# PantoMatrix/PantoMatrix

Hardware: NVIDIA H100
Metric: motion_frames_per_sec (higher is better)
Workload: dtype fp16x3 (two fp16 operand planes, 3 products, f32 accumulate)

## Files before the change

### pantomatrix_b200/csrc/pm_attention_tc.cu

```cuda
#include "pm_common.cuh"
#include "pm_tc_ptx.cuh"
#include "../../include/pm_emage.h"

namespace {

constexpr int T = 64;
constexpr int HD = 192;
constexpr int KB = HD / 64;
constexpr int BLK = T * 128;
constexpr int NTHREADS = 128;
constexpr float P_SCALE = 1024.f;

struct Smem {
  static constexpr int Q = 0;
  static constexpr int K = Q + 2 * KB * BLK;
  static constexpr int V = K + 2 * KB * BLK;
  static constexpr int P = V + 2 * KB * BLK;
  static constexpr int BARS = P + 2 * BLK;
  static constexpr int TOTAL = BARS + (KB + 1) * 8;
};

#ifdef PM_ATTN_TIMING
__device__ unsigned long long pm_attn_stamps[16];
#define AT_STAMP(i) do { if (blockIdx.x == 0 && (threadIdx.x & 31) == 0) pm_attn_stamps[i] = (unsigned long long)clock64(); } while (0)
#else
#define AT_STAMP(i) do {} while (0)
#endif

struct AttnParams {
  int heads, tq, tk;
  int qc0, kc0, vc0;
  float scale;
  float* out; int ldo;
  PmPlanes planes;
};

__global__ void __launch_bounds__(NTHREADS, 1) attention_tc_kernel(const __grid_constant__ CUtensorMap map_q,
                                                                   const __grid_constant__ CUtensorMap map_k,
                                                                   const __grid_constant__ CUtensorMap map_v,
                                                                   const AttnParams p) {
  extern __shared__ __align__(1024) uint8_t smem_raw[];
  uint8_t* sm = reinterpret_cast<uint8_t*>((reinterpret_cast<uintptr_t>(smem_raw) + 1023) & ~uintptr_t(1023));
  const uint32_t sm_u = smem_u32(sm);
  const uint32_t bars = sm_u + Smem::BARS;
  const uint32_t qk_full = bars, v_full = bars + 8 * KB;
  const int warp = threadIdx.x >> 5, lane = threadIdx.x & 31;
  const int b = blockIdx.x / p.heads, h = blockIdx.x % p.heads;
  if (warp == 0) AT_STAMP(0);

  if (threadIdx.x == 0) {
    for (int kb = 0; kb < KB; ++kb) mbar_init(qk_full + 8 * kb, 1);
    mbar_init(v_full, 1);
    asm volatile("fence.mbarrier_init.release.cluster;" ::: "memory");
  }
  __syncthreads();
  if (warp == 0) AT_STAMP(1);
  if (warp == 0) {
    if (elect_one()) {
      asm volatile("prefetch.tensormap [%0];" ::"l"(&map_q) : "memory");
      asm volatile("prefetch.tensormap [%0];" ::"l"(&map_k) : "memory");
      asm volatile("prefetch.tensormap [%0];" ::"l"(&map_v) : "memory");
      for (int kb = 0; kb < KB; ++kb) {
        mbar_expect_tx(qk_full + 8 * kb, 4 * BLK);
        for (int pl = 0; pl < 2; ++pl) {
          tma_load_4d(sm_u + Smem::Q + (pl * KB + kb) * BLK, &map_q, qk_full + 8 * kb, p.qc0 + h * HD + kb * 64, 0, b, pl);
          tma_load_4d(sm_u + Smem::K + (pl * KB + kb) * BLK, &map_k, qk_full + 8 * kb, p.kc0 + h * HD + kb * 64, 0, b, pl);
        }
      }
      mbar_expect_tx(v_full, 2 * KB * BLK);
      for (int pl = 0; pl < 2; ++pl)
        for (int nb = 0; nb < KB; ++nb)
          tma_load_4d(sm_u + Smem::V + (pl * KB + nb) * BLK, &map_v, v_full, p.vc0 + h * HD + nb * 64, 0, b, pl);
    }
    __syncwarp();
  }

  const int r0 = warp * 16 + (lane >> 2), t2 = 2 * (lane & 3);
  const int pa[3] = {0, 1, 0}, pb[3] = {1, 0, 0};

  float sr[32];
#pragma unroll
  for (int i = 0; i < 32; ++i) sr[i] = 0.f;
#pragma unroll
  for (int kb = 0; kb < KB; ++kb) {
    mbar_wait(qk_full + 8 * kb, 0);
    if (warp == 0) AT_STAMP(8 + kb);
    wgmma_fence();
#pragma unroll
// ... 126 lines not shown
}

extern "C" int pm_attention_tc(const uint16_t* Q, long long q_ps, long long q_bs, int ldq, int q_cols, int q_col0,
                               const uint16_t* K, long long k_ps, long long k_bs, int ldk, int k_cols, int k_col0,
                               const uint16_t* V, long long v_ps, long long v_bs, int ldv, int v_cols, int v_col0,
                               float* O, int ldo, int batch, int heads, int tq, int tk, int head_dim,
                               uint16_t* planes, long long p_ps, int p_ld, int p_nsplit, void* stream) {
  PM_REQUIRE(Q && K && V && (O || planes) && batch >= 0 && heads > 0);
  PM_TAKE_FMT(p_nsplit, f16);
  PM_REQUIRE(!planes || (f16 && p_nsplit <= 2));
  PM_REQUIRE(pm_planes_ok(planes, p_ps, p_ld, p_nsplit, heads * head_dim, false));
  if (head_dim != HD || tq > T || tk > T || tq <= 0 || tk <= 0) return PM_EUNSUPPORTED;
  PM_REQUIRE(!O || (ldo & 3) == 0);
  for (const void* ptr : {(const void*)Q, (const void*)K, (const void*)V}) PM_REQUIRE((reinterpret_cast<uintptr_t>(ptr) & 15) == 0);
  PM_REQUIRE((ldq & 7) == 0 && (ldk & 7) == 0 && (ldv & 7) == 0 && (q_ps & 7) == 0 && (k_ps & 7) == 0 && (v_ps & 7) == 0);
  PM_REQUIRE(batch <= 1 || ((q_bs & 7) == 0 && (k_bs & 7) == 0 && (v_bs & 7) == 0));
  PM_REQUIRE(q_col0 >= 0 && k_col0 >= 0 && v_col0 >= 0 && q_col0 + heads * HD <= q_cols && k_col0 + heads * HD <= k_cols &&
             v_col0 + heads * HD <= v_cols && q_cols <= ldq && k_cols <= ldk && v_cols <= ldv);
  if (batch == 0) return PM_OK;
  CUtensorMap mq, mk, mv;
  if (!plane_map(&mq, Q, q_ps, q_bs, ldq, q_cols, tq, batch) || !plane_map(&mk, K, k_ps, k_bs, ldk, k_cols, tk, batch) ||
      !plane_map(&mv, V, v_ps, v_bs, ldv, v_cols, tk, batch))
    return PM_EBADARG;
  AttnParams p;
  p.heads = heads; p.tq = tq; p.tk = tk; p.qc0 = q_col0; p.kc0 = k_col0; p.vc0 = v_col0;
  p.scale = 1.0f / (sqrtf((float)head_dim) * PM_F16_ACT_SCALE * PM_F16_ACT_SCALE);
  p.out = O; p.ldo = ldo;
  p.planes = PmPlanes{reinterpret_cast<__nv_bfloat16*>(planes), p_ps, p_ld, p_nsplit};
  static unsigned long long configured = 0;
  if (pm_first_use_on_device(configured)) {
    cudaError_t e = cudaFuncSetAttribute(attention_tc_kernel, cudaFuncAttributeMaxDynamicSharedMemorySize, (int)kSmem);
    if (e != cudaSuccess) { configured = 0; return (int)e; }
  }
  attention_tc_kernel<<<batch * heads, NTHREADS, kSmem, (cudaStream_t)stream>>>(mq, mk, mv, p);
  PM_LAUNCH_CHECK();
}

#ifdef PM_ATTN_TIMING
extern "C" int pm_attn_timing_read(unsigned long long* host) {
  cudaError_t e = cudaDeviceSynchronize();
  if (e != cudaSuccess) return (int)e;
  return (int)cudaMemcpyFromSymbol(host, pm_attn_stamps, sizeof(unsigned long long) * 16);
}
#endif
```

### pantomatrix_b200/csrc/pm_common.cuh

```cuda
#pragma once
#include <cuda_bf16.h>
#include <cuda_fp16.h>
#include <cuda_runtime.h>
#include <stdint.h>

#define PM_OK 0
#define PM_EBADARG (-1)
#define PM_EUNSUPPORTED (-2)

#define PM_LAUNCH_CHECK()                                  \
  do {                                                     \
    cudaError_t _e = cudaGetLastError();                   \
    return _e == cudaSuccess ? PM_OK : (int)_e;            \
  } while (0)

#define PM_REQUIRE(cond) \
  do {                   \
    if (!(cond)) return PM_EBADARG; \
  } while (0)

static inline int pm_cdiv(long long a, long long b) { return (int)((a + b - 1) / b); }

static inline bool pm_first_use_on_device(unsigned long long& mask) {
  int d = 0;
  if (cudaGetDevice(&d) != cudaSuccess || d < 0 || d >= 64) return true;
  if ((mask >> d) & 1ull) return false;
  mask |= 1ull << d;
  return true;
}

enum PmAct { PM_ACT_NONE = 0, PM_ACT_RELU = 1, PM_ACT_LEAKY = 2 };

__device__ __forceinline__ float pm_act(float v, int act, float slope) {
  if (act == PM_ACT_RELU) return v > 0.f ? v : 0.f;
  if (act == PM_ACT_LEAKY) return v > 0.f ? v : v * slope;
  return v;
}

__device__ __forceinline__ float pm_warp_sum(float v) {
#pragma unroll
  for (int o = 16; o > 0; o >>= 1) v += __shfl_xor_sync(0xffffffffu, v, o);
  return v;
}

__device__ __forceinline__ float pm_warp_max(float v) {
#pragma unroll
  for (int o = 16; o > 0; o >>= 1) v = fmaxf(v, __shfl_xor_sync(0xffffffffu, v, o));
  return v;
}

struct PmPlanes {
  __nv_bfloat16* ptr;
  long long ps;
  int ld;
// ... 99 lines not shown
```

### pantomatrix_b200/csrc/pm_elementwise.cu

```cuda
#include "pm_common.cuh"
#include "../../include/pm_emage.h"

namespace {

constexpr int STEM_ROWS = 192;
constexpr int STEM_THREADS = 256;

template <bool F16>
__device__ __forceinline__ void stem_store_planes2(const PmPlanes& P, long long row, int c, float a, float b) {
  if constexpr (F16) {
    if (P.nsplit == 2) {
      __half* o = reinterpret_cast<__half*>(P.ptr) + row * P.ld + c;
      a *= PM_F16_ACT_SCALE; b *= PM_F16_ACT_SCALE;
      const float a0 = pm_f16_head(a), b0 = pm_f16_head(b);
      *reinterpret_cast<__half2*>(o) = __floats2half2_rn(a0, b0);
      *reinterpret_cast<__half2*>(o + P.ps) = __floats2half2_rn(a - a0, b - b0);
      return;
    }
  }
  pm_store_planes_t<F16>(P, row, c, a);
  pm_store_planes_t<F16>(P, row, c + 1, b);
}

template <int KS, int COUT, bool F16>
// ... 54 lines not shown
      }
    } else {
#pragma unroll
      for (int j = 0; j < 3; ++j) {
#pragma unroll
        for (int k = 0; k < KS; ++k) {
          const float v = xr[j * stride + k];
          acc[j][0] = fmaf(v, wa0[k], acc[j][0]);
          acc[j][1] = fmaf(v, wa1[k], acc[j][1]);
          acc[j][2] = fmaf(v, wb0[k], acc[j][2]);
          acc[j][3] = fmaf(v, wb1[k], acc[j][3]);
        }
      }
    }
#pragma unroll
    for (int j = 0; j < 3; ++j) {
      const int l = l0 + r0 + j;
      if (l >= rows_out) break;
      float a0 = acc[j][0] + ba0, a1 = acc[j][1] + ba1;
      a0 = a0 > 0.f ? a0 : a0 * slope;
      a1 = a1 > 0.f ? a1 : a1 * slope;
      const long long row = (long long)seq * rows_out + l;
      *reinterpret_cast<float2*>(sc + row * COUT + c0) = make_float2(acc[j][2] + bb0, acc[j][3] + bb1);
      if (y1) *reinterpret_cast<float2*>(y1 + row * COUT + c0) = make_float2(a0, a1);
      if (P.ptr) stem_store_planes2<F16>(P, row, c0, a0, a1);
    }
  }
}

template <int VEC, bool F16>
__global__ void __launch_bounds__(256) add_layernorm_kernel(
    const float* __restrict__ x, const float* __restrict__ r, const float* __restrict__ gamma,
    const float* __restrict__ beta, float* __restrict__ out, long long rows, float eps, PmPlanes P) {
  const int lane = threadIdx.x & 31;
  const long long row = (long long)blockIdx.x * (blockDim.x >> 5) + (threadIdx.x >> 5);
  if (row >= rows) return;
  constexpr int CH = VEC * 128;
  const float4* __restrict__ xr = reinterpret_cast<const float4*>(x + row * CH);
  const float4* __restrict__ rr = r ? reinterpret_cast<const float4*>(r + row * CH) : nullptr;
  float4 v[VEC];
  float s = 0.f;
#pragma unroll
  for (int i = 0; i < VEC; ++i) {
    v[i] = xr[lane + 32 * i];
    if (rr) {
      const float4 t = rr[lane + 32 * i];
      v[i].x += t.x; v[i].y += t.y; v[i].z += t.z; v[i].w += t.w;
    }
    s += (v[i].x + v[i].y) + (v[i].z + v[i].w);
  }
  const float mean = pm_warp_sum(s) * (1.f / CH);
  float q = 0.f;
#pragma unroll
  for (int i = 0; i < VEC; ++i) {
    const float a = v[i].x - mean, b = v[i].y - mean, c = v[i].z - mean, d = v[i].w - mean;
    q += (a * a + b * b) + (c * c + d * d);
  }
  const float rstd = rsqrtf(pm_warp_sum(q) * (1.f / CH) + eps);
  const float4* __restrict__ g4 = reinterpret_cast<const float4*>(gamma);
  const float4* __restrict__ b4 = reinterpret_cast<const float4*>(beta);
  float4* __restrict__ o4 = out ? reinterpret_cast<float4*>(out + row * CH) : nullptr;
#pragma unroll
  for (int i = 0; i < VEC; ++i) {
    const float4 g = g4[lane + 32 * i], bb = b4[lane + 32 * i];
    float4 o;
    o.x = (v[i].x - mean) * rstd * g.x + bb.x;
    o.y = (v[i].y - mean) * rstd * g.y + bb.y;
    o.z = (v[i].z - mean) * rstd * g.z + bb.z;
    o.w = (v[i].w - mean) * rstd * g.w + bb.w;
    if (o4) o4[lane + 32 * i] = o;
    if (P.ptr) pm_store_planes4_t<F16>(P, row, (lane + 32 * i) * 4, o);
  }
}

__device__ __forceinline__ float4 pick_row(int code, const float* pe, const float* spk, int b, int t, int ch, int c4) {
  if (code == 1) return reinterpret_cast<const float4*>(pe + (long long)t * ch)[c4];
  if (code == 2) return reinterpret_cast<const float4*>(spk + (long long)b * ch)[c4];
  return make_float4(0.f, 0.f, 0.f, 0.f);
}

template <bool F16>
__global__ void __launch_bounds__(256) add_rows_kernel(
    const float* __restrict__ x, const float* __restrict__ pe, const float* __restrict__ spk,
    int first, int second, float* __restrict__ out, int batch, int rows, int ch, PmPlanes P) {
  const int ch4 = ch >> 2;
  const long long total = (long long)batch * rows * ch4;
  for (long long i = (long long)blockIdx.x * blockDim.x + threadIdx.x; i < total;
       i += (long long)gridDim.x * blockDim.x) {
    const int c4 = (int)(i % ch4);
    const long long bt = i / ch4;
    const int t = (int)(bt % rows), b = (int)(bt / rows);
    float4 v = x ? reinterpret_cast<const float4*>(x)[i] : make_float4(0.f, 0.f, 0.f, 0.f);
    if (first) {
      const float4 a = pick_row(first, pe, spk, b, t, ch, c4);
      v.x += a.x; v.y += a.y; v.z += a.z; v.w += a.w;
    }
    if (second) {
      const float4 a = pick_row(second, pe, spk, b, t, ch, c4);
      v.x += a.x; v.y += a.y; v.z += a.z; v.w += a.w;
    }
    if (out) reinterpret_cast<float4*>(out)[i] = v;
    if (P.ptr) pm_store_planes4_t<F16>(P, bt, c4 * 4, v);
  }
}

template <bool F16>
__global__ void __launch_bounds__(256) add2_kernel(const float* __restrict__ a, long long lda,
                                                   const float* __restrict__ b, long long ldb,
                                                   float* __restrict__ out, long long ldo, long long rows,
                                                   long long ch, long long nv, PmPlanes P) {
  const long long i0 = (long long)blockIdx.x * blockDim.x + threadIdx.x, step = (long long)gridDim.x * blockDim.x;
  for (long long i = i0; i < rows * nv; i += step) {
    const long long r = rows == 1 ? 0 : i / nv, c = (i - r * nv) * 4;
    const float4 u = *reinterpret_cast<const float4*>(a + r * lda + c);
    const float4 v = *reinterpret_cast<const float4*>(b + r * ldb + c);
    const float4 o = make_float4(u.x + v.x, u.y + v.y, u.z + v.z, u.w + v.w);
    if (out) *reinterpret_cast<float4*>(out + r * ldo + c) = o;
    if (P.ptr) pm_store_planes4_t<F16>(P, r, (int)c, o);
  }
  const long long nt = ch - 4 * nv;
  for (long long i = i0; i < rows * nt; i += step) {
    const long long r = i / nt, c = 4 * nv + (i - r * nt);
    const float o = a[r * lda + c] + b[r * ldb + c];
    if (out) out[r * ldo + c] = o;
    if (P.ptr) pm_store_planes_t<F16>(P, r, (int)c, o);
  }
}

template <bool F16>
__global__ void __launch_bounds__(256) window_input_kernel(
    const float* __restrict__ motion, const float* __restrict__ mask, const float* __restrict__ seed,
    const float* __restrict__ mask_embedding, float* __restrict__ out,
    int batch, int total_len, int start, int win_len, int pre, int ch, long long seed_bs, PmPlanes P) {
  const long long total = (long long)batch * win_len * ch;
  for (long long i = (long long)blockIdx.x * blockDim.x + threadIdx.x; i < total;
       i += (long long)gridDim.x * blockDim.x) {
    const int c = (int)(i % ch);
    const long long bf = i / ch;
    const int f = (int)(bf % win_len), b = (int)(bf / win_len);
    const long long src = ((long long)b * total_len + start + f) * ch + c;
    float m = mask ? mask[src] : 1.f;
    float v = motion ? motion[src] : ((c < ch - 7 && (c % 6 == 0 || c % 6 == 4)) ? 1.f : 0.f);
    if (f < pre) {
      if (m != 0.f && seed) v = seed[(long long)b * seed_bs + (long long)f * ch + c];
      m = 0.f;
    }
    const float o = (m == 1.f) ? mask_embedding[c] : v;
    if (out) out[i] = o;
    if (P.ptr) pm_store_planes_t<F16>(P, bf, c, o);
  }
}

inline int grid_for(long long work, int threads) {
  long long g = (work + threads - 1) / threads;
  const long long cap = 148LL * 16;
  return (int)(g < 1 ? 1 : (g > cap ? cap : g));
}

}

extern "C" int pm_wav_stem_f32(const float* audio, long long a_bs, long long a_ws, int batch, int windows,
                               int n_samples, const float* w1, const float* b1, const float* wd,
                               const float* bd, int cout, int ksize, int stride, int pad, int rows_out,
                               float slope, float* y1, float* sc,
                               uint16_t* planes, long long p_ps, int p_ld, int p_nsplit, void* stream) {
  PM_REQUIRE(audio && w1 && b1 && wd && bd && sc && (y1 || planes));
  PM_REQUIRE(batch > 0 && windows > 0 && n_samples > 0 && cout > 0 && stride > 0 && rows_out > 0);
  PM_TAKE_FMT(p_nsplit, f16);
  PM_REQUIRE(pm_planes_ok(planes, p_ps, p_ld, p_nsplit, cout, false));
  PM_REQUIRE(!planes || ((p_ld & 1) == 0 && (p_ps & 1) == 0 && (reinterpret_cast<uintptr_t>(planes) & 3) == 0));
  PM_REQUIRE((reinterpret_cast<uintptr_t>(sc) & 7) == 0 && (!y1 || (reinterpret_cast<uintptr_t>(y1) & 7) == 0));
  if (ksize != 15 || (cout != 32 && cout != 64)) return PM_EUNSUPPORTED;
  PM_REQUIRE((long long)batch * windows <= 65535);
  const size_t smem = (size_t)((STEM_ROWS - 1) * stride + ksize) * sizeof(float);
  PM_REQUIRE(smem <= 48 * 1024);
  const PmPlanes P{reinterpret_cast<__nv_bfloat16*>(planes), p_ps, p_ld, planes ? p_nsplit : 0};
  dim3 grid(pm_cdiv(rows_out, STEM_ROWS), batch * windows);
  cudaStream_t st = (cudaStream_t)stream;
#define PM_STEM(CO, F)                                                                                          \
  wav_stem_kernel<15, CO, F><<<grid, STEM_THREADS, smem, st>>>(audio, a_bs, a_ws, batch, n_samples, w1, b1, wd, bd, \
                                                               stride, pad, rows_out, slope, y1, sc, P)
  if (cout == 64) { if (f16) PM_STEM(64, true); else PM_STEM(64, false); }
  else { if (f16) PM_STEM(32, true); else PM_STEM(32, false); }
#undef PM_STEM
  PM_LAUNCH_CHECK();
}

extern "C" int pm_add_layernorm_f32(const float* x, const float* r, const float* gamma, const float* beta,
                                    float* out, long long rows, int ch, float eps,
                                    uint16_t* planes, long long p_ps, int p_ld, int p_nsplit, void* stream) {
  PM_REQUIRE(x && gamma && beta && (out || planes) && rows >= 0);
  PM_TAKE_FMT(p_nsplit, f16);
  PM_REQUIRE(pm_planes_ok(planes, p_ps, p_ld, p_nsplit, ch, true));
  const PmPlanes P{reinterpret_cast<__nv_bfloat16*>(planes), p_ps, p_ld, p_nsplit};
  if (rows == 0) return PM_OK;
  const int warps = 8;
  const unsigned grid = (unsigned)((rows + warps - 1) / warps);
  cudaStream_t st = (cudaStream_t)stream;
  switch (ch) {
    case 256:
      if (f16) add_layernorm_kernel<2, true><<<grid, warps * 32, 0, st>>>(x, r, gamma, beta, out, rows, eps, P);
      else add_layernorm_kernel<2, false><<<grid, warps * 32, 0, st>>>(x, r, gamma, beta, out, rows, eps, P);
      break;
    case 512:
      if (f16) add_layernorm_kernel<4, true><<<grid, warps * 32, 0, st>>>(x, r, gamma, beta, out, rows, eps, P);
      else add_layernorm_kernel<4, false><<<grid, warps * 32, 0, st>>>(x, r, gamma, beta, out, rows, eps, P);
      break;
    case 768:
      if (f16) add_layernorm_kernel<6, true><<<grid, warps * 32, 0, st>>>(x, r, gamma, beta, out, rows, eps, P);
      else add_layernorm_kernel<6, false><<<grid, warps * 32, 0, st>>>(x, r, gamma, beta, out, rows, eps, P);
      break;
    case 1024:
      if (f16) add_layernorm_kernel<8, true><<<grid, warps * 32, 0, st>>>(x, r, gamma, beta, out, rows, eps, P);
      else add_layernorm_kernel<8, false><<<grid, warps * 32, 0, st>>>(x, r, gamma, beta, out, rows, eps, P);
      break;
    default: return PM_EUNSUPPORTED;
  }
  PM_LAUNCH_CHECK();
}

extern "C" int pm_add_rows_f32(const float* x, const float* pe, const float* spk, int first, int second,
                               float* out, int batch, int rows, int ch,
                               uint16_t* planes, long long p_ps, int p_ld, int p_nsplit, void* stream) {
  PM_REQUIRE((out || planes) && batch >= 0 && rows >= 0 && ch > 0 && (ch & 3) == 0);
  PM_TAKE_FMT(p_nsplit, f16);
  PM_REQUIRE(pm_planes_ok(planes, p_ps, p_ld, p_nsplit, ch, true));
  const PmPlanes P{reinterpret_cast<__nv_bfloat16*>(planes), p_ps, p_ld, p_nsplit};
  PM_REQUIRE(first >= 0 && first <= 2 && second >= 0 && second <= 2);
  PM_REQUIRE((first != 1 && second != 1) || pe);
  PM_REQUIRE((first != 2 && second != 2) || spk);
  const long long total = (long long)batch * rows * (ch >> 2);
  if (total == 0) return PM_OK;
  if (f16) add_rows_kernel<true><<<grid_for(total, 256), 256, 0, (cudaStream_t)stream>>>(x, pe, spk, first, second, out,
                                                                                  batch, rows, ch, P);
  else add_rows_kernel<false><<<grid_for(total, 256), 256, 0, (cudaStream_t)stream>>>(x, pe, spk, first, second, out,
                                                                               batch, rows, ch, P);
  PM_LAUNCH_CHECK();
}

extern "C" int pm_add2_strided_f32(const float* a, long long lda, const float* b, long long ldb, float* out,
                                   long long ldo, long long rows, long long ch,
                                   uint16_t* planes, long long p_ps, int p_ld, int p_nsplit, void* stream) {
  PM_REQUIRE(a && b && (out || planes) && rows >= 0 && ch > 0);
  PM_REQUIRE(rows <= 1 || (lda >= ch && ldb >= ch && (!out || ldo >= ch)));
  PM_REQUIRE(!planes || ((ch & 3) == 0 && ch <= 0x7fffffffLL));
  PM_TAKE_FMT(p_nsplit, f16);
  PM_REQUIRE(pm_planes_ok(planes, p_ps, p_ld, p_nsplit, (int)(planes ? ch : 1), true));
  const PmPlanes P{reinterpret_cast<__nv_bfloat16*>(planes), p_ps, p_ld, p_nsplit};
  if (rows == 0) return PM_OK;
  const auto a16 = [](const void* p) { return (reinterpret_cast<uintptr_t>(p) & 15) == 0; };
  const bool vec = a16(a) && a16(b) && (!out || a16(out)) &&
                   (rows == 1 || ((lda & 3) == 0 && (ldb & 3) == 0 && (!out || (ldo & 3) == 0)));
  const long long nv = vec ? ch / 4 : 0;
  const int grid = grid_for(rows * (nv + (ch - 4 * nv)), 256);
  cudaStream_t st = (cudaStream_t)stream;
  if (f16) add2_kernel<true><<<grid, 256, 0, st>>>(a, lda, b, ldb, out, ldo, rows, ch, nv, P);
  else add2_kernel<false><<<grid, 256, 0, st>>>(a, lda, b, ldb, out, ldo, rows, ch, nv, P);
  PM_LAUNCH_CHECK();
}

extern "C" int pm_add2_f32(const float* a, const float* b, float* out, long long n, int ch,
                           uint16_t* planes, long long p_ps, int p_ld, int p_nsplit, void* stream) {
  PM_REQUIRE(a && b && (out || planes) && n >= 0);
  PM_REQUIRE(!planes || (ch > 0 && (ch & 3) == 0 && n % ch == 0));
  if (n == 0) return PM_OK;
  const long long rows = planes ? n / ch : 1, cols = planes ? ch : n;
  return pm_add2_strided_f32(a, cols, b, cols, out, cols, rows, cols, planes, p_ps, p_ld, p_nsplit, stream);
}

extern "C" int pm_window_input_f32(const float* motion, const float* mask, const float* seed,
                                   const float* mask_embedding, float* out, int batch, int total_len,
                                   int start, int win_len, int pre, int ch, long long seed_bs,
                                   uint16_t* planes, long long p_ps, int p_ld, int p_nsplit, void* stream) {
  PM_REQUIRE(mask_embedding && (out || planes));
  PM_TAKE_FMT(p_nsplit, f16);
  PM_REQUIRE(pm_planes_ok(planes, p_ps, p_ld, p_nsplit, ch, false));
  const PmPlanes P{reinterpret_cast<__nv_bfloat16*>(planes), p_ps, p_ld, p_nsplit};
  PM_REQUIRE(batch >= 0 && win_len >= 0 && start >= 0 && start + win_len <= total_len && pre >= 0 && ch > 0);
  const long long total = (long long)batch * win_len * ch;
  if (total == 0) return PM_OK;
  if (f16) window_input_kernel<true><<<grid_for(total, 256), 256, 0, (cudaStream_t)stream>>>(
      motion, mask, seed, mask_embedding, out, batch, total_len, start, win_len, pre, ch, seed_bs, P);
  else window_input_kernel<false><<<grid_for(total, 256), 256, 0, (cudaStream_t)stream>>>(
      motion, mask, seed, mask_embedding, out, batch, total_len, start, win_len, pre, ch, seed_bs, P);
  PM_LAUNCH_CHECK();
}
```

### pantomatrix_b200/csrc/pm_tapgemm_tc.cu

```cuda
#include <cuda.h>
#include <stdio.h>
#include <stdlib.h>

#include <cstring>
#include "pm_common.cuh"
#include "../../include/pm_emage.h"


namespace {

constexpr int BM = 128;
constexpr int BK = 64;
constexpr int MMA_K = 16;
constexpr int A_TILE_BYTES = BM * BK * 2;
constexpr int PRODUCER_THREADS = 128;
constexpr int CONSUMER_THREADS = 256;
constexpr int NUM_THREADS = PRODUCER_THREADS + CONSUMER_THREADS;
constexpr int PRODUCER_REGS = 40, CONSUMER_REGS = 232;
static_assert(PRODUCER_THREADS * PRODUCER_REGS + CONSUMER_THREADS * CONSUMER_REGS == (65536 / NUM_THREADS & ~7) * NUM_THREADS,
              "the setmaxnreg split must use exactly the launch's register pool");
constexpr int STAMP_WARP = PRODUCER_THREADS / 32;
constexpr int MAX_STAGES = 8;
constexpr int RING_KB = 200;

// ... 74 lines not shown
  const int warp = threadIdx.x >> 5, lane = threadIdx.x & 31;
  if (warp == STAMP_WARP) PM_STAMP(0);
  const int l0 = blockIdx.x * p.R;
  const int n0 = blockIdx.y * BN;
  const int b0 = blockIdx.z * p.NB;
  const int n_iter = p.taps * p.kblocks;

  if (threadIdx.x == 0) {
    asm volatile("prefetch.tensormap [%0];" ::"l"(&map_a) : "memory");
    asm volatile("prefetch.tensormap [%0];" ::"l"(&map_w) : "memory");
    for (int s = 0; s < p.stages; ++s) {
      mbar_init(smem_u32(&full_bar[s]), 1);
      mbar_init(smem_u32(&empty_bar[s]), 2);
    }
    asm volatile("fence.mbarrier_init.release.cluster;" ::: "memory");
  }
  __syncthreads();
  if (warp == STAMP_WARP) PM_STAMP(1);

  if (warp < PRODUCER_THREADS / 32) {
    setmaxnreg_dec<PRODUCER_REGS>();
    if (warp == 1 && lane == 0 && p.prefetch) {
      const long long ncta = (long long)gridDim.x * gridDim.y * gridDim.z;
      const long long cta = ((long long)blockIdx.z * gridDim.y + blockIdx.y) * gridDim.x + blockIdx.x;
      long long share = ((p.prefetch_bytes + ncta - 1) / ncta + 127) & ~127LL;
      long long off = cta * share;
      long long end = off + share < p.prefetch_bytes ? off + share : p.prefetch_bytes;
      end &= ~15LL;
      for (; off < end; off += 16384) {
        const uint32_t n = (uint32_t)(end - off < 16384 ? end - off : 16384);
        asm volatile("cp.async.bulk.prefetch.L2.global [%0], %1;" ::"l"(p.prefetch + off), "r"(n) : "memory");
      }
    }
    if (warp != 0) return;
    const uint32_t tx = (uint32_t)stage_bytes;
    int s = 0, tap = 0, kb = 0;
    uint32_t ph = 0;
    for (int it = 0; it < n_iter; ++it) {
      mbar_wait_fast(smem_u32(&empty_bar[s]), ph ^ 1u);
      if (elect_one()) {
        const uint32_t bar = smem_u32(&full_bar[s]);
        uint8_t* st = tiles + (size_t)s * stage_bytes;
        mbar_expect_tx(bar, tx);
        for (int pl = 0; pl < p.nsplit; ++pl) {
          tma_load_4d(smem_u32(st + pl * A_TILE_BYTES), &map_a, bar, kb * BK, l0 + tap - p.pad, b0, pl);
          tma_load_3d(smem_u32(st + p.nsplit * A_TILE_BYTES + pl * W_TILE_BYTES), &map_w, bar, kb * BK, tap * p.w_rows + n0, pl);
        }
      }
      __syncwarp();
      if (++s == p.stages) { s = 0; ph ^= 1u; }
      if (++kb == p.kblocks) { kb = 0; ++tap; }
    }
    return;
  }

  setmaxnreg_inc<CONSUMER_REGS>();
  const int ct = threadIdx.x - PRODUCER_THREADS;
  const int wg = ct >> 7;
  float acc0[NACC], acc1[NACC], accc[NACC];
#pragma unroll
  for (int i = 0; i < NACC; ++i) { acc0[i] = 0.f; acc1[i] = 0.f; accc[i] = 0.f; }
  {
    const uint32_t tiles_u32 = smem_u32(tiles);
    int s = 0;
    uint32_t ph = 0;
    int prev = -1;
    auto kblock = [&](float (&main)[NACC]) {
      mbar_wait_fast(smem_u32(&full_bar[s]), ph);
      if (prev < 0 && warp == STAMP_WARP) PM_STAMP(2);
      const uint32_t a_base = tiles_u32 + (uint32_t)s * (uint32_t)stage_bytes + (uint32_t)wg * (64 * 128);
      const uint32_t w_base = tiles_u32 + (uint32_t)s * (uint32_t)stage_bytes + (uint32_t)(NSPLIT * A_TILE_BYTES);
      wgmma_fence();
      mma_kblock<BN, F16, NSPLIT>(main, accc, gmma_desc(GMMA_DESC_K_SW128, a_base), gmma_desc(GMMA_DESC_K_SW128, w_base));
      wgmma_commit();
      wgmma_wait<1>();
      if (prev >= 0 && ct % 128 == 0) mbar_arrive(smem_u32(&empty_bar[prev]));
      prev = s;
      if (++s == p.stages) { s = 0; ph ^= 1u; }
    };
    int it = 0;
    for (; it + 1 < n_iter; it += 2) {
      kblock(acc0);
      kblock(acc1);
    }
    if (it < n_iter) kblock(acc0);
    if (warp == STAMP_WARP) PM_STAMP(3);
    wgmma_wait<0>();
    if (warp == STAMP_WARP) PM_STAMP(4);
    wgmma_fence_regs(acc0);
    wgmma_fence_regs(acc1);
    wgmma_fence_regs(accc);
  }
  named_bar_sync(1, CONSUMER_THREADS);
  {
    const int wq = warp & 3, t4 = lane & 3;
    const int r0 = wg * 64 + wq * 16 + (lane >> 2);
    float* stg = reinterpret_cast<float*>(tiles);
#pragma unroll
    for (int i = 0; i < NACC / 4; ++i) {
      const int c = 8 * i + 2 * t4;
#pragma unroll
      for (int h = 0; h < 2; ++h) {
        float v0 = acc0[4 * i + 2 * h] + acc1[4 * i + 2 * h];
        float v1 = acc0[4 * i + 2 * h + 1] + acc1[4 * i + 2 * h + 1];
        v0 += accc[4 * i + 2 * h];
        v1 += accc[4 * i + 2 * h + 1];
        if constexpr (F16) { v0 *= p.acc_scale; v1 *= p.acc_scale; }
        *reinterpret_cast<float2*>(stg + (r0 + 8 * h) * ST + c) = make_float2(v0, v1);
      }
    }
  }
  named_bar_sync(1, CONSUMER_THREADS);

  const bool vec_f = p.out_f32 && ((p.ldo & 3) == 0) && ((reinterpret_cast<uintptr_t>(p.out_f32) & 15) == 0) && ((p.o_bs & 3) == 0);
  const bool vec_r = p.residual && ((p.ldr & 3) == 0) && ((reinterpret_cast<uintptr_t>(p.residual) & 15) == 0) && ((p.r_bs & 3) == 0);
  const bool vec_b = p.out_bf16 && ((p.ldob & 3) == 0) && ((reinterpret_cast<uintptr_t>(p.out_bf16) & 7) == 0) &&
                     ((p.ob_bs & 3) == 0) && ((p.ob_ps & 3) == 0);
  const bool all_vec = (!p.out_f32 || vec_f) && (!p.residual || vec_r) && (!p.out_bf16 || vec_b);
  const float act_slope = p.act == PM_ACT_NONE ? 1.f : (p.act == PM_ACT_RELU ? 0.f : p.slope);
  const int r_shift = 31 - __clz(p.R);
  constexpr int C4 = BN / 4;
  const float* stg = reinterpret_cast<const float*>(tiles);
#pragma unroll 1
  for (int item = ct; item < BM * C4; item += CONSUMER_THREADS) {
    const int rt = item / C4, c = (item % C4) * 4;
    const int b = b0 + (rt >> r_shift), l = l0 + (rt & (p.R - 1));
    const int n = n0 + c;
    if (b >= p.batch || l >= p.rows_out || n >= p.cout) continue;
    const float4 x4 = *reinterpret_cast<const float4*>(stg + rt * ST + c);
    const long long of = (long long)b * p.o_bs + (long long)l * p.ldo;
    const long long orr = (long long)b * p.r_bs + (long long)l * p.ldr;
    const PmPlanes P{p.out_bf16 ? p.out_bf16 + (long long)b * p.ob_bs + (long long)l * p.ldob : nullptr,
                     p.ob_ps, p.ldob, p.out_nsplit};
    if (all_vec && n + 4 <= p.cout) {
      float4 x = x4;
      if (p.bias) { x.x += __ldg(p.bias + n); x.y += __ldg(p.bias + n + 1); x.z += __ldg(p.bias + n + 2); x.w += __ldg(p.bias + n + 3); }
      if (p.residual) {
        const float4 t = *reinterpret_cast<const float4*>(p.residual + orr + n);
        x.x += t.x; x.y += t.y; x.z += t.z; x.w += t.w;
      }
      x.x = x.x < 0.f ? (n < p.act_cols ? act_slope : 1.f) * x.x : x.x;
      x.y = x.y < 0.f ? (n + 1 < p.act_cols ? act_slope : 1.f) * x.y : x.y;
      x.z = x.z < 0.f ? (n + 2 < p.act_cols ? act_slope : 1.f) * x.z : x.z;
      x.w = x.w < 0.f ? (n + 3 < p.act_cols ? act_slope : 1.f) * x.w : x.w;
      if (p.out_f32) *reinterpret_cast<float4*>(p.out_f32 + of + n) = x;
      if (P.ptr) pm_store_planes4_t<F16>(P, 0, n, x);
    } else {
      const float xs[4] = {x4.x, x4.y, x4.z, x4.w};
#pragma unroll
      for (int k = 0; k < 4; ++k) {
        if (n + k >= p.cout) break;
        float y = xs[k];
        if (p.bias) y += __ldg(p.bias + n + k);
        if (p.residual) y += p.residual[orr + n + k];
        y = y < 0.f ? (n + k < p.act_cols ? act_slope : 1.f) * y : y;
        if (p.out_f32) p.out_f32[of + n + k] = y;
        if (P.ptr) pm_store_planes_t<F16>(P, 0, n + k, y);
      }
    }
  }
  if (warp == STAMP_WARP) PM_STAMP(5);
#ifdef PM_TC_TIMING
  named_bar_sync(1, CONSUMER_THREADS);
#endif
  if (warp == STAMP_WARP) PM_STAMP(6);
}

template <bool VEC, bool F16>
__global__ void __launch_bounds__(256) split_bf16_kernel(const float* __restrict__ x, long long x_bs, int ldx, int rows,
                                                         int ch, __nv_bfloat16* __restrict__ out, long long o_ps,
                                                         long long o_bs, int ldo, int nsplit) {
  const int b = blockIdx.y;
  const float* __restrict__ xb = x + (long long)b * x_bs;
  __nv_bfloat16* __restrict__ ob = out + (long long)b * o_bs;
  if (VEC) {
    const int ch4 = ch >> 2;
    const long long total = (long long)rows * ch4;
    for (long long i = (long long)blockIdx.x * blockDim.x + threadIdx.x; i < total; i += (long long)gridDim.x * blockDim.x) {
      const int r = (int)(i / ch4), c4 = (int)(i - (long long)r * ch4);
      const float4 v = *reinterpret_cast<const float4*>(xb + (long long)r * ldx + 4 * c4);
      const PmPlanes P{ob, o_ps, ldo, nsplit};
      pm_store_planes4_t<F16>(P, r, 4 * c4, v);
    }
  } else {
    const long long total = (long long)rows * ch;
    for (long long i = (long long)blockIdx.x * blockDim.x + threadIdx.x; i < total; i += (long long)gridDim.x * blockDim.x) {
      const int r = (int)(i / ch), c = (int)(i - (long long)r * ch);
      const PmPlanes P{ob, o_ps, ldo, nsplit};
      pm_store_planes_t<F16>(P, r, c, xb[(long long)r * ldx + c]);
    }
  }
}

template <int BN, bool F16, int NSPLIT>
int launch(const CUtensorMap& ma, const CUtensorMap& mw, TcParams& p, dim3 grid, cudaStream_t st) {
  const int stage_bytes = p.nsplit * (A_TILE_BYTES + BN * BK * 2);
  int stages = RING_KB * 1024 / stage_bytes;
  if (stages > MAX_STAGES) stages = MAX_STAGES;
  if (stages < 2) return PM_EUNSUPPORTED;
  p.stages = stages;
  const int staging = BM * (BN + 8) * 4;
  const size_t ring = (size_t)stages * stage_bytes > (size_t)staging ? (size_t)stages * stage_bytes : (size_t)staging;
  const size_t smem = ring + 1024  + 2 * MAX_STAGES * sizeof(uint64_t);
  static unsigned long long configured = 0;
  if (pm_first_use_on_device(configured)) {
    cudaError_t e = cudaFuncSetAttribute(tapgemm_tc_kernel<BN, F16, NSPLIT>, cudaFuncAttributeMaxDynamicSharedMemorySize, 227 * 1024);
    if (e != cudaSuccess) { configured = 0; return (int)e; }
  }
  tapgemm_tc_kernel<BN, F16, NSPLIT><<<grid, NUM_THREADS, smem, st>>>(ma, mw, p);
  PM_LAUNCH_CHECK();
}

template <int BN>
int launch_fmt(const CUtensorMap& ma, const CUtensorMap& mw, TcParams& p, dim3 grid, cudaStream_t st, bool f16) {
  if (f16) {
    if (p.nsplit == 1) return launch<BN, true, 1>(ma, mw, p, grid, st);
    if (p.nsplit == 2) return launch<BN, true, 2>(ma, mw, p, grid, st);
    return launch<BN, true, 3>(ma, mw, p, grid, st);
  }
  if (p.nsplit == 1) return launch<BN, false, 1>(ma, mw, p, grid, st);
  if (p.nsplit == 2) return launch<BN, false, 2>(ma, mw, p, grid, st);
  return launch<BN, false, 3>(ma, mw, p, grid, st);
}

int pick_bn(long long row_tiles, int cout, int w_rows, int sms) {
  if (cout <= 64 || w_rows % 128) return 64;
  const long long waves64 = (row_tiles * pm_cdiv(cout, 64) + sms - 1) / sms;
  const long long waves128 = (row_tiles * pm_cdiv(cout, 128) + sms - 1) / sms;
  return waves128 * 14 <= waves64 * 10 ? 128 : 64;
}

}

extern "C" int pm_tapgemm_tc(const uint16_t* A, long long a_ps, long long a_bs, int lda, int batch, int rows_in, int cin,
                             const uint16_t* W, long long w_ps, int w_rows, int ldw, int taps, int pad, int nsplit,
                             const float* bias, int rows_out, int cout,
                             const float* residual, long long r_bs, int ldr,
                             int act, int act_cols, float slope, float acc_scale,
                             float* out_f32, long long o_bs, int ldo,
                             uint16_t* out_bf16, long long ob_ps, long long ob_bs, int ldob, int out_nsplit,
                             const void* prefetch, long long prefetch_bytes, void* stream) {
  PM_REQUIRE(A && W && (out_f32 || out_bf16));
// ... 63 lines not shown
}

#ifdef PM_TC_TIMING
extern "C" int pm_tc_timing_reset() {
  cudaError_t e = cudaDeviceSynchronize();
  if (e != cudaSuccess) return (int)e;
  void* d = nullptr;
  e = cudaGetSymbolAddress(&d, pm_tc_stamps);
  if (e != cudaSuccess) return (int)e;
  return (int)cudaMemset(d, 0, sizeof(unsigned long long) * 4096 * 8);
}
extern "C" int pm_tc_timing_read(unsigned long long* host) {
  cudaError_t e = cudaDeviceSynchronize();
  if (e != cudaSuccess) return (int)e;
  return (int)cudaMemcpyFromSymbol(host, pm_tc_stamps, sizeof(unsigned long long) * 4096 * 8);
}
#endif

extern "C" int pm_split_bf16(const float* x, long long x_bs, int ldx, int batch, int rows, int ch,
                             uint16_t* out, long long o_ps, long long o_bs, int ldo, int nsplit, void* stream) {
  PM_TAKE_FMT(nsplit, f16);
  PM_REQUIRE(x && out && batch >= 0 && rows >= 0 && ch > 0 && ldx >= ch && ldo >= ch && nsplit >= 1 && nsplit <= 3);
  if ((long long)batch * rows == 0) return PM_OK;
  PM_REQUIRE(batch <= 65535);
  const bool vec = (ch & 3) == 0 && (ldx & 3) == 0 && (x_bs & 3) == 0 && (ldo & 3) == 0 && (o_bs & 3) == 0 &&
                   (o_ps & 3) == 0 && (reinterpret_cast<uintptr_t>(x) & 15) == 0 && (reinterpret_cast<uintptr_t>(out) & 7) == 0;
  const long long work = (long long)rows * (vec ? ch / 4 : ch);
  long long gx = (work + 255) / 256;
  const long long cap = batch >= 132 * 4 ? 1 : (132 * 8 + batch - 1) / batch;
  if (gx > cap) gx = cap;
  dim3 grid((unsigned)gx, batch);
  __nv_bfloat16* o = reinterpret_cast<__nv_bfloat16*>(out);
  cudaStream_t st = (cudaStream_t)stream;
  if (f16) {
    if (vec) split_bf16_kernel<true, true><<<grid, 256, 0, st>>>(x, x_bs, ldx, rows, ch, o, o_ps, o_bs, ldo, nsplit);
    else split_bf16_kernel<false, true><<<grid, 256, 0, st>>>(x, x_bs, ldx, rows, ch, o, o_ps, o_bs, ldo, nsplit);
  } else {
    if (vec) split_bf16_kernel<true, false><<<grid, 256, 0, st>>>(x, x_bs, ldx, rows, ch, o, o_ps, o_bs, ldo, nsplit);
    else split_bf16_kernel<false, false><<<grid, 256, 0, st>>>(x, x_bs, ldx, rows, ch, o, o_ps, o_bs, ldo, nsplit);
  }
  PM_LAUNCH_CHECK();
}
```

Measured before the change: 304,700.

## Enable programmatic dependent launch across kernels and prefetch GEMM weights before wait

Launches the attention, elementwise, split and tap-GEMM kernels with programmatic stream serialization and adds griddepcontrol wait/trigger calls. Each kernel's prologue (barrier init, tensormap prefetch, weight TMA loads for the first stages) can then overlap the tail of the previous kernel. The GEMM producer issues weight tile loads before waiting on the upstream kernel, because weights do not depend on prior outputs. The epilogue is also restructured so each thread keeps one column, hoisting the bias load and batching the residual loads. The risk is a correctness hazard if any prologue touches data written by the predecessor, and the extra launch-attribute overhead.

```diff
diff --git a/pantomatrix_b200/csrc/pm_attention_tc.cu b/pantomatrix_b200/csrc/pm_attention_tc.cu
--- a/pantomatrix_b200/csrc/pm_attention_tc.cu
+++ b/pantomatrix_b200/csrc/pm_attention_tc.cu
@@ -54,6 +54,8 @@
     asm volatile("fence.mbarrier_init.release.cluster;" ::: "memory");
   }
   __syncthreads();
+  pm_pdl_wait();
+  pm_pdl_trigger();
   if (warp == 0) AT_STAMP(1);
   if (warp == 0) {
     if (elect_one()) {
@@ -246,7 +248,7 @@
     cudaError_t e = cudaFuncSetAttribute(attention_tc_kernel, cudaFuncAttributeMaxDynamicSharedMemorySize, (int)kSmem);
     if (e != cudaSuccess) { configured = 0; return (int)e; }
   }
-  attention_tc_kernel<<<batch * heads, NTHREADS, kSmem, (cudaStream_t)stream>>>(mq, mk, mv, p);
+  pm_launch_pdl(attention_tc_kernel, dim3(batch * heads), dim3(NTHREADS), kSmem, (cudaStream_t)stream, mq, mk, mv, p);
   PM_LAUNCH_CHECK();
 }
 
diff --git a/pantomatrix_b200/csrc/pm_common.cuh b/pantomatrix_b200/csrc/pm_common.cuh
--- a/pantomatrix_b200/csrc/pm_common.cuh
+++ b/pantomatrix_b200/csrc/pm_common.cuh
@@ -20,6 +20,25 @@
   } while (0)
 
 static inline int pm_cdiv(long long a, long long b) { return (int)((a + b - 1) / b); }
+
+__device__ __forceinline__ void pm_pdl_wait() { asm volatile("griddepcontrol.wait;" ::: "memory"); }
+__device__ __forceinline__ void pm_pdl_trigger() { asm volatile("griddepcontrol.launch_dependents;" ::: "memory"); }
+
+template <typename... KArgs, typename... Args>
+static inline cudaError_t pm_launch_pdl(void (*kernel)(KArgs...), dim3 grid, dim3 block, size_t smem, cudaStream_t st,
+                                        Args&&... args) {
+  cudaLaunchAttribute attr[1];
+  attr[0].id = cudaLaunchAttributeProgrammaticStreamSerialization;
+  attr[0].val.programmaticStreamSerializationAllowed = 1;
+  cudaLaunchConfig_t cfg = {};
+  cfg.gridDim = grid;
+  cfg.blockDim = block;
+  cfg.dynamicSmemBytes = smem;
+  cfg.stream = st;
+  cfg.attrs = attr;
+  cfg.numAttrs = 1;
+  return cudaLaunchKernelEx(&cfg, kernel, static_cast<Args&&>(args)...);
+}
 
 static inline bool pm_first_use_on_device(unsigned long long& mask) {
   int d = 0;
diff --git a/pantomatrix_b200/csrc/pm_elementwise.cu b/pantomatrix_b200/csrc/pm_elementwise.cu
--- a/pantomatrix_b200/csrc/pm_elementwise.cu
+++ b/pantomatrix_b200/csrc/pm_elementwise.cu
@@ -110,6 +110,8 @@
 __global__ void __launch_bounds__(256) add_layernorm_kernel(
     const float* __restrict__ x, const float* __restrict__ r, const float* __restrict__ gamma,
     const float* __restrict__ beta, float* __restrict__ out, long long rows, float eps, PmPlanes P) {
+  pm_pdl_wait();
+  pm_pdl_trigger();
   const int lane = threadIdx.x & 31;
   const long long row = (long long)blockIdx.x * (blockDim.x >> 5) + (threadIdx.x >> 5);
   if (row >= rows) return;
@@ -161,6 +163,8 @@
 __global__ void __launch_bounds__(256) add_rows_kernel(
     const float* __restrict__ x, const float* __restrict__ pe, const float* __restrict__ spk,
     int first, int second, float* __restrict__ out, int batch, int rows, int ch, PmPlanes P) {
+  pm_pdl_wait();
+  pm_pdl_trigger();
   const int ch4 = ch >> 2;
   const long long total = (long long)batch * rows * ch4;
   for (long long i = (long long)blockIdx.x * blockDim.x + threadIdx.x; i < total;
@@ -187,6 +191,8 @@
                                                    const float* __restrict__ b, long long ldb,
                                                    float* __restrict__ out, long long ldo, long long rows,
                                                    long long ch, long long nv, PmPlanes P) {
+  pm_pdl_wait();
+  pm_pdl_trigger();
   const long long i0 = (long long)blockIdx.x * blockDim.x + threadIdx.x, step = (long long)gridDim.x * blockDim.x;
   for (long long i = i0; i < rows * nv; i += step) {
     const long long r = rows == 1 ? 0 : i / nv, c = (i - r * nv) * 4;
@@ -210,6 +216,8 @@
     const float* __restrict__ motion, const float* __restrict__ mask, const float* __restrict__ seed,
     const float* __restrict__ mask_embedding, float* __restrict__ out,
     int batch, int total_len, int start, int win_len, int pre, int ch, long long seed_bs, PmPlanes P) {
+  pm_pdl_wait();
+  pm_pdl_trigger();
   const long long total = (long long)batch * win_len * ch;
   for (long long i = (long long)blockIdx.x * blockDim.x + threadIdx.x; i < total;
        i += (long long)gridDim.x * blockDim.x) {
@@ -275,25 +283,23 @@
   const int warps = 8;
   const unsigned grid = (unsigned)((rows + warps - 1) / warps);
   cudaStream_t st = (cudaStream_t)stream;
+  void (*kern)(const float*, const float*, const float*, const float*, float*, long long, float, PmPlanes);
   switch (ch) {
     case 256:
-      if (f16) add_layernorm_kernel<2, true><<<grid, warps * 32, 0, st>>>(x, r, gamma, beta, out, rows, eps, P);
-      else add_layernorm_kernel<2, false><<<grid, warps * 32, 0, st>>>(x, r, gamma, beta, out, rows, eps, P);
+      kern = f16 ? add_layernorm_kernel<2, true> : add_layernorm_kernel<2, false>;
       break;
     case 512:
-      if (f16) add_layernorm_kernel<4, true><<<grid, warps * 32, 0, st>>>(x, r, gamma, beta, out, rows, eps, P);
-      else add_layernorm_kernel<4, false><<<grid, warps * 32, 0, st>>>(x, r, gamma, beta, out, rows, eps, P);
+      kern = f16 ? add_layernorm_kernel<4, true> : add_layernorm_kernel<4, false>;
       break;
     case 768:
-      if (f16) add_layernorm_kernel<6, true><<<grid, warps * 32, 0, st>>>(x, r, gamma, beta, out, rows, eps, P);
-      else add_layernorm_kernel<6, false><<<grid, warps * 32, 0, st>>>(x, r, gamma, beta, out, rows, eps, P);
+      kern = f16 ? add_layernorm_kernel<6, true> : add_layernorm_kernel<6, false>;
       break;
     case 1024:
-      if (f16) add_layernorm_kernel<8, true><<<grid, warps * 32, 0, st>>>(x, r, gamma, beta, out, rows, eps, P);
-      else add_layernorm_kernel<8, false><<<grid, warps * 32, 0, st>>>(x, r, gamma, beta, out, rows, eps, P);
+      kern = f16 ? add_layernorm_kernel<8, true> : add_layernorm_kernel<8, false>;
       break;
     default: return PM_EUNSUPPORTED;
   }
+  pm_launch_pdl(kern, dim3(grid), dim3(warps * 32), 0, st, x, r, gamma, beta, out, rows, eps, P);
   PM_LAUNCH_CHECK();
 }
 
@@ -309,10 +315,8 @@
   PM_REQUIRE((first != 2 && second != 2) || spk);
   const long long total = (long long)batch * rows * (ch >> 2);
   if (total == 0) return PM_OK;
-  if (f16) add_rows_kernel<true><<<grid_for(total, 256), 256, 0, (cudaStream_t)stream>>>(x, pe, spk, first, second, out,
-                                                                                  batch, rows, ch, P);
-  else add_rows_kernel<false><<<grid_for(total, 256), 256, 0, (cudaStream_t)stream>>>(x, pe, spk, first, second, out,
-                                                                               batch, rows, ch, P);
+  pm_launch_pdl(f16 ? add_rows_kernel<true> : add_rows_kernel<false>, dim3(grid_for(total, 256)), dim3(256), 0,
+                (cudaStream_t)stream, x, pe, spk, first, second, out, batch, rows, ch, P);
   PM_LAUNCH_CHECK();
 }
 
@@ -332,8 +336,8 @@
   const long long nv = vec ? ch / 4 : 0;
   const int grid = grid_for(rows * (nv + (ch - 4 * nv)), 256);
   cudaStream_t st = (cudaStream_t)stream;
-  if (f16) add2_kernel<true><<<grid, 256, 0, st>>>(a, lda, b, ldb, out, ldo, rows, ch, nv, P);
-  else add2_kernel<false><<<grid, 256, 0, st>>>(a, lda, b, ldb, out, ldo, rows, ch, nv, P);
+  pm_launch_pdl(f16 ? add2_kernel<true> : add2_kernel<false>, dim3(grid), dim3(256), 0, st, a, lda, b, ldb, out, ldo, rows,
+                ch, nv, P);
   PM_LAUNCH_CHECK();
 }
 
@@ -357,9 +361,8 @@
   PM_REQUIRE(batch >= 0 && win_len >= 0 && start >= 0 && start + win_len <= total_len && pre >= 0 && ch > 0);
   const long long total = (long long)batch * win_len * ch;
   if (total == 0) return PM_OK;
-  if (f16) window_input_kernel<true><<<grid_for(total, 256), 256, 0, (cudaStream_t)stream>>>(
-      motion, mask, seed, mask_embedding, out, batch, total_len, start, win_len, pre, ch, seed_bs, P);
-  else window_input_kernel<false><<<grid_for(total, 256), 256, 0, (cudaStream_t)stream>>>(
-      motion, mask, seed, mask_embedding, out, batch, total_len, start, win_len, pre, ch, seed_bs, P);
-  PM_LAUNCH_CHECK();
-}
+  pm_launch_pdl(f16 ? window_input_kernel<true> : window_input_kernel<false>, dim3(grid_for(total, 256)), dim3(256), 0,
+                (cudaStream_t)stream, motion, mask, seed, mask_embedding, out, batch, total_len, start, win_len, pre, ch,
+                seed_bs, P);
+  PM_LAUNCH_CHECK();
+}
diff --git a/pantomatrix_b200/csrc/pm_tapgemm_tc.cu b/pantomatrix_b200/csrc/pm_tapgemm_tc.cu
--- a/pantomatrix_b200/csrc/pm_tapgemm_tc.cu
+++ b/pantomatrix_b200/csrc/pm_tapgemm_tc.cu
@@ -130,8 +130,25 @@
         asm volatile("cp.async.bulk.prefetch.L2.global [%0], %1;" ::"l"(p.prefetch + off), "r"(n) : "memory");
       }
     }
-    if (warp != 0) return;
+    if (warp != 0) {
+      pm_pdl_wait();
+      return;
+    }
     const uint32_t tx = (uint32_t)stage_bytes;
+    const int pre = n_iter < p.stages ? n_iter : p.stages;
+    if (elect_one()) {
+      int tap = 0, kb = 0;
+      for (int it = 0; it < pre; ++it) {
+        const uint32_t bar = smem_u32(&full_bar[it]);
+        uint8_t* st = tiles + (size_t)it * stage_bytes;
+        mbar_expect_tx(bar, tx);
+        for (int pl = 0; pl < p.nsplit; ++pl)
+          tma_load_3d(smem_u32(st + p.nsplit * A_TILE_BYTES + pl * W_TILE_BYTES), &map_w, bar, kb * BK, tap * p.w_rows + n0, pl);
+        if (++kb == p.kblocks) { kb = 0; ++tap; }
+      }
+    }
+    __syncwarp();
+    pm_pdl_wait();
     int s = 0, tap = 0, kb = 0;
     uint32_t ph = 0;
     for (int it = 0; it < n_iter; ++it) {
@@ -139,10 +156,11 @@
       if (elect_one()) {
         const uint32_t bar = smem_u32(&full_bar[s]);
         uint8_t* st = tiles + (size_t)s * stage_bytes;
-        mbar_expect_tx(bar, tx);
+        if (it >= pre) mbar_expect_tx(bar, tx);
         for (int pl = 0; pl < p.nsplit; ++pl) {
           tma_load_4d(smem_u32(st + pl * A_TILE_BYTES), &map_a, bar, kb * BK, l0 + tap - p.pad, b0, pl);
-          tma_load_3d(smem_u32(st + p.nsplit * A_TILE_BYTES + pl * W_TILE_BYTES), &map_w, bar, kb * BK, tap * p.w_rows + n0, pl);
+          if (it >= pre)
+            tma_load_3d(smem_u32(st + p.nsplit * A_TILE_BYTES + pl * W_TILE_BYTES), &map_w, bar, kb * BK, tap * p.w_rows + n0, pl);
         }
       }
       __syncwarp();
@@ -153,6 +171,7 @@
   }
 
   setmaxnreg_inc<CONSUMER_REGS>();
+  pm_pdl_wait();
   const int ct = threadIdx.x - PRODUCER_THREADS;
   const int wg = ct >> 7;
   float acc0[NACC], acc1[NACC], accc[NACC];
@@ -183,6 +202,7 @@
     }
     if (it < n_iter) kblock(acc0);
     if (warp == STAMP_WARP) PM_STAMP(3);
+    pm_pdl_trigger();
     wgmma_wait<0>();
     if (warp == STAMP_WARP) PM_STAMP(4);
     wgmma_fence_regs(acc0);
@@ -218,32 +238,51 @@
   const float act_slope = p.act == PM_ACT_NONE ? 1.f : (p.act == PM_ACT_RELU ? 0.f : p.slope);
   const int r_shift = 31 - __clz(p.R);
   constexpr int C4 = BN / 4;
+  constexpr int ITEMS = BM * C4 / CONSUMER_THREADS, RSTEP = CONSUMER_THREADS / C4;
+  static_assert(CONSUMER_THREADS % C4 == 0, "a thread's items share one column");
   const float* stg = reinterpret_cast<const float*>(tiles);
+  const int c = (ct % C4) * 4, n = n0 + c, rt0 = ct / C4;
+  if (all_vec && n + 4 <= p.cout) {
+    float4 bv = make_float4(0.f, 0.f, 0.f, 0.f);
+    if (p.bias) bv = make_float4(__ldg(p.bias + n), __ldg(p.bias + n + 1), __ldg(p.bias + n + 2), __ldg(p.bias + n + 3));
+    float4 res[ITEMS];
+#pragma unroll
+    for (int j = 0; j < ITEMS; ++j) {
+      const int rt = rt0 + j * RSTEP;
+      const int b = b0 + (rt >> r_shift), l = l0 + (rt & (p.R - 1));
+      res[j] = make_float4(0.f, 0.f, 0.f, 0.f);
+      if (p.residual && b < p.batch && l < p.rows_out)
+        res[j] = *reinterpret_cast<const float4*>(p.residual + (long long)b * p.r_bs + (long long)l * p.ldr + n);
+    }
+#pragma unroll
+    for (int j = 0; j < ITEMS; ++j) {
+      const int rt = rt0 + j * RSTEP;
+      const int b = b0 + (rt >> r_shift), l = l0 + (rt & (p.R - 1));
+      if (b < p.batch && l < p.rows_out) {
+        float4 x = *reinterpret_cast<const float4*>(stg + rt * ST + c);
+        if (p.bias) { x.x += bv.x; x.y += bv.y; x.z += bv.z; x.w += bv.w; }
+        if (p.residual) { x.x += res[j].x; x.y += res[j].y; x.z += res[j].z; x.w += res[j].w; }
+        x.x = x.x < 0.f ? (n < p.act_cols ? act_slope : 1.f) * x.x : x.x;
+        x.y = x.y < 0.f ? (n + 1 < p.act_cols ? act_slope : 1.f) * x.y : x.y;
+        x.z = x.z < 0.f ? (n + 2 < p.act_cols ? act_slope : 1.f) * x.z : x.z;
+        x.w = x.w < 0.f ? (n + 3 < p.act_cols ? act_slope : 1.f) * x.w : x.w;
+        if (p.out_f32) *reinterpret_cast<float4*>(p.out_f32 + (long long)b * p.o_bs + (long long)l * p.ldo + n) = x;
+        if (p.out_bf16) {
+          const PmPlanes P{p.out_bf16 + (long long)b * p.ob_bs + (long long)l * p.ldob, p.ob_ps, p.ldob, p.out_nsplit};
+          pm_store_planes4_t<F16>(P, 0, n, x);
+        }
+      }
+    }
+  } else if (n < p.cout) {
 #pragma unroll 1
-  for (int item = ct; item < BM * C4; item += CONSUMER_THREADS) {
-    const int rt = item / C4, c = (item % C4) * 4;
-    const int b = b0 + (rt >> r_shift), l = l0 + (rt & (p.R - 1));
-    const int n = n0 + c;
-    if (b >= p.batch || l >= p.rows_out || n >= p.cout) continue;
-    const float4 x4 = *reinterpret_cast<const float4*>(stg + rt * ST + c);
-    const long long of = (long long)b * p.o_bs + (long long)l * p.ldo;
-    const long long orr = (long long)b * p.r_bs + (long long)l * p.ldr;
-    const PmPlanes P{p.out_bf16 ? p.out_bf16 + (long long)b * p.ob_bs + (long long)l * p.ldob : nullptr,
-                     p.ob_ps, p.ldob, p.out_nsplit};
-    if (all_vec && n + 4 <= p.cout) {
-      float4 x = x4;
-      if (p.bias) { x.x += __ldg(p.bias + n); x.y += __ldg(p.bias + n + 1); x.z += __ldg(p.bias + n + 2); x.w += __ldg(p.bias + n + 3); }
-      if (p.residual) {
-        const float4 t = *reinterpret_cast<const float4*>(p.residual + orr + n);
-        x.x += t.x; x.y += t.y; x.z += t.z; x.w += t.w;
-      }
-      x.x = x.x < 0.f ? (n < p.act_cols ? act_slope : 1.f) * x.x : x.x;
-      x.y = x.y < 0.f ? (n + 1 < p.act_cols ? act_slope : 1.f) * x.y : x.y;
-      x.z = x.z < 0.f ? (n + 2 < p.act_cols ? act_slope : 1.f) * x.z : x.z;
-      x.w = x.w < 0.f ? (n + 3 < p.act_cols ? act_slope : 1.f) * x.w : x.w;
-      if (p.out_f32) *reinterpret_cast<float4*>(p.out_f32 + of + n) = x;
-      if (P.ptr) pm_store_planes4_t<F16>(P, 0, n, x);
-    } else {
+    for (int rt = rt0; rt < BM; rt += RSTEP) {
+      const int b = b0 + (rt >> r_shift), l = l0 + (rt & (p.R - 1));
+      if (b >= p.batch || l >= p.rows_out) continue;
+      const float4 x4 = *reinterpret_cast<const float4*>(stg + rt * ST + c);
+      const long long of = (long long)b * p.o_bs + (long long)l * p.ldo;
+      const long long orr = (long long)b * p.r_bs + (long long)l * p.ldr;
+      const PmPlanes P{p.out_bf16 ? p.out_bf16 + (long long)b * p.ob_bs + (long long)l * p.ldob : nullptr,
+                       p.ob_ps, p.ldob, p.out_nsplit};
       const float xs[4] = {x4.x, x4.y, x4.z, x4.w};
 #pragma unroll
       for (int k = 0; k < 4; ++k) {
@@ -268,6 +307,8 @@
 __global__ void __launch_bounds__(256) split_bf16_kernel(const float* __restrict__ x, long long x_bs, int ldx, int rows,
                                                          int ch, __nv_bfloat16* __restrict__ out, long long o_ps,
                                                          long long o_bs, int ldo, int nsplit) {
+  pm_pdl_wait();
+  pm_pdl_trigger();
   const int b = blockIdx.y;
   const float* __restrict__ xb = x + (long long)b * x_bs;
   __nv_bfloat16* __restrict__ ob = out + (long long)b * o_bs;
@@ -305,7 +346,7 @@
     cudaError_t e = cudaFuncSetAttribute(tapgemm_tc_kernel<BN, F16, NSPLIT>, cudaFuncAttributeMaxDynamicSharedMemorySize, 227 * 1024);
     if (e != cudaSuccess) { configured = 0; return (int)e; }
   }
-  tapgemm_tc_kernel<BN, F16, NSPLIT><<<grid, NUM_THREADS, smem, st>>>(ma, mw, p);
+  pm_launch_pdl(tapgemm_tc_kernel<BN, F16, NSPLIT>, grid, dim3(NUM_THREADS), smem, st, ma, mw, p);
   PM_LAUNCH_CHECK();
 }
 
@@ -435,12 +476,8 @@
   dim3 grid((unsigned)gx, batch);
   __nv_bfloat16* o = reinterpret_cast<__nv_bfloat16*>(out);
   cudaStream_t st = (cudaStream_t)stream;
-  if (f16) {
-    if (vec) split_bf16_kernel<true, true><<<grid, 256, 0, st>>>(x, x_bs, ldx, rows, ch, o, o_ps, o_bs, ldo, nsplit);
-    else split_bf16_kernel<false, true><<<grid, 256, 0, st>>>(x, x_bs, ldx, rows, ch, o, o_ps, o_bs, ldo, nsplit);
-  } else {
-    if (vec) split_bf16_kernel<true, false><<<grid, 256, 0, st>>>(x, x_bs, ldx, rows, ch, o, o_ps, o_bs, ldo, nsplit);
-    else split_bf16_kernel<false, false><<<grid, 256, 0, st>>>(x, x_bs, ldx, rows, ch, o, o_ps, o_bs, ldo, nsplit);
-  }
+  const auto kern = f16 ? (vec ? split_bf16_kernel<true, true> : split_bf16_kernel<false, true>)
+                        : (vec ? split_bf16_kernel<true, false> : split_bf16_kernel<false, false>);
+  pm_launch_pdl(kern, grid, dim3(256), 0, st, x, x_bs, ldx, rows, ch, o, o_ps, o_bs, ldo, nsplit);
   PM_LAUNCH_CHECK();
 }
```

New measurement: 311,600 (median of 6 runs). 2.2% higher.
